# ignacio-rocco/detectorch

Hardware: AMD Instinct MI355X
Metric: images/sec Mask R-CNN R-50-FPN 1333x800 (region-proposal hot path) (higher is better)
Workload: dtype f32

## Files before the change

detectorch_amd/csrc/roi_align.hip:

```cpp
#include <stdlib.h>

#include <type_traits>

#include "roi_align_common.h"

namespace dtc {

constexpr int kRoiAlignThreads = 256;
constexpr int kMaxTableEntries = 2048;

__device__ __forceinline__ void build_axis_tables(AxisEntry* tab, const RoiHead& hd, const dtc_feat_level& L, int ny, int nx,
                                                  int ymul = 1, int xmul = 1) {
  for (int t = threadIdx.x; t < ny + nx; t += kRoiAlignThreads) {
    const bool is_y = t < ny;
    const int u = is_y ? t : t - ny, g = is_y ? hd.gh : hd.gw, mul = is_y ? ymul : xmul;
    AxisEntry e = make_axis(is_y ? hd.sh : hd.sw, is_y ? hd.bin_h : hd.bin_w, u / g, u % g, g, is_y ? L.height : L.width);
    e.lo *= mul; e.hi *= mul;
    tab[t] = e;
  }
}

template <typename TIn, typename TOut, bool FROM_TABLE>
__device__ __forceinline__ void gather_outputs(const RoiHead& hd, const dtc_feat_level& L, const AxisEntry* ytab, const AxisEntry* xtab,
                                               const TIn* base, TOut* out, int nc, int pooled_w, int bins) {
// ... 503 lines not shown
      } else {
      for (int iy = 0; iy < gh; iy++) {
        const AxisEntry y = tab_ok ? ytab[ph * gh + iy] : [&] { AxisEntry e = make_axis(sh, bin_h, ph, iy, gh, L.height); e.lo *= (int)L.stride_h; e.hi *= (int)L.stride_h; return e; }();
        for (int ix = 0; ix < gw; ix++) {
          const AxisEntry x = tab_ok ? xtab[pw * gw + ix] : [&] { AxisEntry e = make_axis(sw, bin_w, pw, ix, gw, L.width); e.lo *= (int)L.stride_w; e.hi *= (int)L.stride_w; return e; }();
          const float w1 = y.h * x.h, w2 = y.h * x.l, w3 = y.l * x.h, w4 = y.l * x.l;
          float4 v1, v2, v3, v4;
          if (vec) {
            v1 = load4(base + y.lo + x.lo); v2 = load4(base + y.lo + x.hi);
            v3 = load4(base + y.hi + x.lo); v4 = load4(base + y.hi + x.hi);
          } else {
            const TIn* t1 = base + y.lo + x.lo; const TIn* t2 = base + y.lo + x.hi;
            const TIn* t3 = base + y.hi + x.lo; const TIn* t4 = base + y.hi + x.hi;
            const int nv = nc - 4 * q;
            v1 = make_float4(to_f32<TIn>(t1[0]), nv > 1 ? to_f32<TIn>(t1[1]) : 0.f, nv > 2 ? to_f32<TIn>(t1[2]) : 0.f, nv > 3 ? to_f32<TIn>(t1[3]) : 0.f);
            v2 = make_float4(to_f32<TIn>(t2[0]), nv > 1 ? to_f32<TIn>(t2[1]) : 0.f, nv > 2 ? to_f32<TIn>(t2[2]) : 0.f, nv > 3 ? to_f32<TIn>(t2[3]) : 0.f);
            v3 = make_float4(to_f32<TIn>(t3[0]), nv > 1 ? to_f32<TIn>(t3[1]) : 0.f, nv > 2 ? to_f32<TIn>(t3[2]) : 0.f, nv > 3 ? to_f32<TIn>(t3[3]) : 0.f);
            v4 = make_float4(to_f32<TIn>(t4[0]), nv > 1 ? to_f32<TIn>(t4[1]) : 0.f, nv > 2 ? to_f32<TIn>(t4[2]) : 0.f, nv > 3 ? to_f32<TIn>(t4[3]) : 0.f);
          }
          a0 += w1 * v1.x + w2 * v2.x + w3 * v3.x + w4 * v4.x;
          a1 += w1 * v1.y + w2 * v2.y + w3 * v3.y + w4 * v4.y;
          a2 += w1 * v1.z + w2 * v2.z + w3 * v3.z + w4 * v4.z;
          a3 += w1 * v1.w + w2 * v2.w + w3 * v3.w + w4 * v4.w;
        }
      }
      }
      float* so = slab + (4 * q) * bins + bin;
      if (inv_count != 0.f) { so[0] = a0 * inv_count; so[bins] = a1 * inv_count; so[2 * bins] = a2 * inv_count; so[3 * bins] = a3 * inv_count; }
      else { so[0] = fdiv(a0, count); so[bins] = fdiv(a1, count); so[2 * bins] = fdiv(a2, count); so[3 * bins] = fdiv(a3, count); }
    }
  }
  __syncthreads();
  store_slab_vec<TOut, kRoiAlignThreads>(out, slab, nc * bins, tid);
}

const RoiAlignKnobs& roi_align_knobs() {
  static const RoiAlignKnobs knobs = [] {
    RoiAlignKnobs k;
    const auto first_not_0 = [](const char* name, bool dflt) { const char* e = getenv(name); return e ? e[0] != '0' : dflt; };
    const auto is_set = [](const char* name) { return getenv(name) != nullptr; };
    const auto number = [](const char* name, int dflt) { const char* e = getenv(name); return e ? atoi(e) : dflt; };
    const auto in_range = [&](const char* name, int lo, int hi, int dflt) { const int v = number(name, dflt); return v >= lo && v <= hi ? v : dflt; };
    k.tile = first_not_0("DTC_ROIALIGN_TILE", true);
    k.map = first_not_0("DTC_ROIALIGN_MAP", true);
    k.general = is_set("DTC_ROIALIGN_GENERAL");
    k.nhwc_direct = !is_set("DTC_ROIALIGN_NO_NHWC_DIRECT");
    k.nhwc16 = first_not_0("DTC_RA_NHWC16", true);
    k.nhwc_direct32 = first_not_0("DTC_RA_NHWC_DIRECT32", true);
    k.xcd = !is_set("DTC_RA_NO_XCD");
    k.cts64 = !is_set("DTC_RA_NO_CTS64");
    const int cb = number("DTC_RA_TILE_CHBLOCK", 0);
    if (cb >= 4 && (cb & 3) == 0) k.tile_ch_block = cb;
    k.tile_cb_major = number("DTC_RA_TILE_CBMAJOR", 1) != 0;
    k.tile_lds16_kb = in_range("DTC_RA_TILE_LDS16_KB", 36, 156, 0);
    k.map_prep = number("DTC_RA_MAP_PREP", 1) != 0;
    k.map_pitch = first_not_0("DTC_RA_MAP_PITCH", true);
    k.nhwc_lds = number("DTC_RA_NHWC_LDS", 1) != 0;
    k.nhwc_lds_kb = in_range("DTC_RA_NHWC_LDS_KB", 24, 160, 0);
    k.nhwc_pipe = in_range("DTC_RA_NHWC_PIPE", 0, 2, 1);
    return k;
  }();
  return knobs;
}

constexpr int kLdsKernelBytes = 52 * 1024;

template <typename TIn, typename TOut, int CB>
static int launch_nhwc_cb(const RoiAlignParams& p, hipStream_t stream) {
  const size_t smem = (size_t)kLdsTableFloats * 4 + (size_t)CB * p.pooled_h * p.pooled_w * 4 + 16;
  if (raise_lds_once<roi_align_fwd_nhwc<TIn, TOut, CB>>() != DTC_OK) return DTC_ELAUNCH;
  const int nct = ceil_div(p.channels, CB);
  hipLaunchKernelGGL((roi_align_fwd_nhwc<TIn, TOut, CB>), dim3((unsigned)p.n_rois * nct), dim3(kRoiAlignThreads), smem, stream, p);
  DTC_CHECK_LAUNCH();
  return DTC_OK;
}

template <typename TIn, typename TOut>
static int launch_nhwc(const RoiAlignParams& p, hipStream_t stream) {
  if (p.n_rois == 0) return DTC_OK;
  if constexpr (sizeof(TIn) == 2) {
    if (p.pooled_h * p.pooled_w > 64 && p.channels % 32 == 0) return launch_nhwc_cb<TIn, TOut, 32>(p, stream);
  }
  return launch_nhwc_cb<TIn, TOut, 64>(p, stream);
}

template <typename TIn, typename TOut>
static int launch_lds(const RoiAlignParams& p, hipStream_t stream) {
  if (p.n_rois == 0) return DTC_OK;
  if (raise_lds_once<roi_align_fwd_lds<TIn, TOut>>() != DTC_OK) return DTC_ELAUNCH;
  const int nct = ceil_div(p.channels, p.ch_block);
  hipLaunchKernelGGL((roi_align_fwd_lds<TIn, TOut>), dim3((unsigned)p.n_rois * nct), dim3(kRoiAlignThreads), kLdsKernelBytes, stream, p,
                     kLdsKernelBytes / 4);
  DTC_CHECK_LAUNCH();
  return DTC_OK;
}

template <typename TIn, typename TOut>
static int launch_general(const RoiAlignParams& p, hipStream_t stream) {
  if (p.n_rois == 0) return DTC_OK;
  int entries = p.sampling_ratio > 0 ? (p.pooled_h + p.pooled_w) * p.sampling_ratio : kMaxTableEntries;
  if (entries > kMaxTableEntries) entries = kMaxTableEntries;
  size_t smem = (size_t)entries * sizeof(AxisEntry);
  dim3 grid(p.n_rois, ceil_div(p.channels, p.ch_tile));
  hipLaunchKernelGGL((roi_align_fwd_general<TIn, TOut>), grid, dim3(kRoiAlignThreads), smem, stream, p);
  DTC_CHECK_LAUNCH();
  return DTC_OK;
// ... 102 lines not shown
```

detectorch_amd/csrc/roi_align_common.h:

```cpp
#pragma once
#include "dtc_common.h"
#include "wave_ops.h"

namespace dtc {

struct RoiAlignParams {
  dtc_feat_level lv[DTC_MAX_LEVELS];
  const float* rois;
  const int32_t* roi_levels;
  const int32_t* roi_order;
  const float* roi_desc;
  void* out;
  int n_levels, channels, roi_cols, n_rois, pooled_h, pooled_w, sampling_ratio, ch_tile;
  int ch_block;
  int cts64;
  int xcd_remap;
  const void* prep = nullptr;
};

constexpr int kXcds = 8;
__device__ __forceinline__ int xcd_work_item(int b, int n, int enabled) {
  if (!enabled || n < 2 * kXcds) return b;
  const int x = b % kXcds, j = b / kXcds;
  const int q = n / kXcds, r = n - q * kXcds;
// ... 94 lines not shown
  const f32x2 w2 = {w, w};
  acc = __builtin_elementwise_fma(v, w2, acc);
}
template <> __device__ __forceinline__ void fma_pair16<float>(f32x2&, uint32_t, float) {}

__device__ __forceinline__ float4 load4(const float* p) { return *reinterpret_cast<const float4*>(p); }
__device__ __forceinline__ float4 load4(const __half* p) { return f16x4_to_f32(*reinterpret_cast<const uint2*>(p)); }
__device__ __forceinline__ float4 load4(const bf16_t* p) { return bf16x4_to_f32(*reinterpret_cast<const uint2*>(p)); }

template <typename TOut> __device__ __forceinline__ void store4(TOut* d, float4 v);
template <> __device__ __forceinline__ void store4<float>(float* d, float4 v) { store_stream16(d, v); }
template <> __device__ __forceinline__ void store4<__half>(__half* d, float4 v) {
  const __half2 a = __floats2half2_rn(v.x, v.y), b = __floats2half2_rn(v.z, v.w);
  store_stream8(d, *reinterpret_cast<const uint32_t*>(&a), *reinterpret_cast<const uint32_t*>(&b));
}
template <> __device__ __forceinline__ void store4<bf16_t>(bf16_t* d, float4 v) {
  store_stream8(d, (uint32_t)from_f32<bf16_t>(v.x).bits | ((uint32_t)from_f32<bf16_t>(v.y).bits << 16),
                (uint32_t)from_f32<bf16_t>(v.z).bits | ((uint32_t)from_f32<bf16_t>(v.w).bits << 16));
}

template <typename TOut, int THREADS>
__device__ __forceinline__ void zero_outputs(TOut* out, int n, int tid) {
  for (int o = tid; o < n; o += THREADS) out[o] = from_f32<TOut>(0.f);
}

template <typename T> struct dtype_tag { typedef T type; };
template <typename Tag> using tag_type = typename Tag::type;
template <typename F>
inline int dispatch_io_pair(int in_dtype, int out_dtype, F&& f) {
  if (in_dtype == DTC_F32 && out_dtype == DTC_F32) return f(dtype_tag<float>{}, dtype_tag<float>{});
  if (in_dtype == DTC_F16 && out_dtype == DTC_F32) return f(dtype_tag<__half>{}, dtype_tag<float>{});
  if (in_dtype == DTC_F16 && out_dtype == DTC_F16) return f(dtype_tag<__half>{}, dtype_tag<__half>{});
  if (in_dtype == DTC_F32 && out_dtype == DTC_F16) return f(dtype_tag<float>{}, dtype_tag<__half>{});
  if (in_dtype == DTC_BF16 && out_dtype == DTC_F32) return f(dtype_tag<bf16_t>{}, dtype_tag<float>{});
  if (in_dtype == DTC_BF16 && out_dtype == DTC_BF16) return f(dtype_tag<bf16_t>{}, dtype_tag<bf16_t>{});
  if (in_dtype == DTC_F32 && out_dtype == DTC_BF16) return f(dtype_tag<float>{}, dtype_tag<bf16_t>{});
  return DTC_EUNSUPPORTED;
}
inline bool io_pair_supported(int in_dtype, int out_dtype) {
  return dispatch_io_pair(in_dtype, out_dtype, [](auto, auto) { return (int)DTC_OK; }) == DTC_OK;
}

struct RoiAlignKnobs {
  bool tile = true;
  bool map = true;
  bool general = false;
  bool nhwc_direct = true;
  bool nhwc16 = true;
  bool nhwc_direct32 = true;
  bool xcd = true;
  bool cts64 = true;
  int tile_ch_block = 0;
  int tile_cb_major = 1;
  int tile_lds16_kb = 0;
  bool map_prep = true;
  bool map_pitch = true;
  int nhwc_lds = 1;
  int nhwc_lds_kb = 0;
  int nhwc_pipe = 1;
};
const RoiAlignKnobs& roi_align_knobs();

bool roi_align_tile_supported(const RoiAlignParams& p, int in_dtype, int out_dtype);
int launch_roi_align_tile(const RoiAlignParams& p, int in_dtype, int out_dtype, hipStream_t stream);
bool roi_align_map_supported(const RoiAlignParams& p, int in_dtype, int out_dtype);
int launch_roi_align_map(const RoiAlignParams& p, int in_dtype, int out_dtype, hipStream_t stream);
void roi_align_set_exact(int exact);
int roi_align_get_exact();
size_t roi_align_map_workspace_bytes(int n_rois);
int launch_roi_align_map_ws(const RoiAlignParams& p, int in_dtype, int out_dtype, void* workspace, size_t workspace_bytes, hipStream_t stream);

bool roi_align_nhwc_lds_supported(const RoiAlignParams& p, int in_dtype, int out_dtype);
int launch_roi_align_nhwc_lds(const RoiAlignParams& p, int in_dtype, int out_dtype, hipStream_t stream);

bool roi_align_nhwc16_supported(const RoiAlignParams& p, int in_dtype, int out_dtype);
int launch_roi_align_nhwc16(const RoiAlignParams& p, int in_dtype, int out_dtype, hipStream_t stream);

}
```

detectorch_amd/csrc/roi_align_tile.hip:

```cpp

#include <type_traits>

#include "roi_align_common.h"

namespace dtc {

constexpr int kTileMaxK = 32;
constexpr int kTileRoiBytes = 48, kTileGroupBytes = 32;
constexpr int kTileHdrBytes = kTileMaxK * (kTileRoiBytes + kTileGroupBytes) + 16;
template <int NT> struct TileShape;
template <> struct TileShape<256> { static constexpr int kUnits = 8, kWaves = 3, kLdsKB = 52, kWaves16 = 4, kLds16KB = 38; };

struct TileRoi {
  int lvl, b, x0, x1, y0, y1, r, valid;
  float sh, sw, bin_h, bin_w;
};
static_assert(sizeof(TileRoi) == kTileRoiBytes, "TileRoi layout");
struct TileGroup { int first, count, kind, x0, x1, y0, y1, pad; };
enum { kGrpPool = 0, kGrpZero = 1, kGrpAbsent = 2, kGrpGather = 3 };

__device__ __forceinline__ __amdgpu_buffer_rsrc_t make_srd(const void* base) {
  return __builtin_amdgcn_make_buffer_rsrc(const_cast<void*>(base), 0, 0xffffffff, 0x00020000);
}
template <typename TIn> struct Piece4;
template <> struct Piece4<float> {
  typedef float4 Raw;
  static __device__ __forceinline__ Raw raw(__amdgpu_buffer_rsrc_t r, uint32_t voff, uint32_t soff) {
    const u32x4 v = __builtin_amdgcn_raw_buffer_load_b128(r, voff, soff, 0);
    return make_float4(__uint_as_float(v.x), __uint_as_float(v.y), __uint_as_float(v.z), __uint_as_float(v.w));
  }
};
template <> struct Piece4<__half> {
  typedef u32x2 Raw;
  static __device__ __forceinline__ Raw raw(__amdgpu_buffer_rsrc_t r, uint32_t voff, uint32_t soff) { return __builtin_amdgcn_raw_buffer_load_b64(r, voff, soff, 0); }
};
template <> struct Piece4<bf16_t> {
  typedef u32x2 Raw;
  static __device__ __forceinline__ Raw raw(__amdgpu_buffer_rsrc_t r, uint32_t voff, uint32_t soff) { return __builtin_amdgcn_raw_buffer_load_b64(r, voff, soff, 0); }
};

template <typename TIn> struct TileLds { typedef float T; static constexpr int kSlot = 16, kShift = 4; };
template <> struct TileLds<__half> { typedef uint16_t T; static constexpr int kSlot = 8, kShift = 3; };
template <> struct TileLds<bf16_t> { typedef uint16_t T; static constexpr int kSlot = 8, kShift = 3; };

template <typename TIn, int NT> struct TileBounds { static constexpr int kWaves = TileShape<NT>::kWaves; };
template <int NT> struct TileBounds<__half, NT> { static constexpr int kWaves = TileShape<NT>::kWaves16; };
template <int NT> struct TileBounds<bf16_t, NT> { static constexpr int kWaves = TileShape<NT>::kWaves16; };

__device__ __forceinline__ int tile_phys(int px) { return px + (px >> 3); }

struct TileItem {
  int a[2][2][4];
  float yl[2], yh[2], xl[2], xh[2];
  bool on;
};

enum { kStageScalar = 0, kStageVec = 1, kStageVecUnaligned = 2 };

struct TileGeom {
  int first, count;
  int y0, x0a, ngx, npos;
  int plane;
  int nq_pass;
  int mode;
};

template <typename TIn, typename TOut, int NT, bool FUSED>
__device__ __forceinline__ void tile_passes(const RoiAlignParams& p, const dtc_feat_level& L, const TIn* fbase, int c0, int nc,
                                            int bins, float* slab, typename TileLds<TIn>::T* win, const TileRoi* troi, const TileGeom& g,
                                            const TileItem& it, int rl, int bin) {
  constexpr int NW = NT / 64;
  constexpr int U = TileShape<NT>::kUnits;
  typedef typename TileLds<TIn>::T TL;
  constexpr bool L16 = sizeof(TL) == 2;
  constexpr int SB = TileLds<TIn>::kSlot;
  const int tid = threadIdx.x, lane = tid & 63, wv = tid >> 6, pl = lane & 15, cl = (lane >> 4) & 3;
  const int npos = g.npos, ngx = g.ngx, plane = g.plane, nq_pass = g.nq_pass;
  const int nchunk = (npos + 15) >> 4;
  const int KC = ceil_div(nchunk, NW);
  const float rinv = 1.0f / (float)ngx;
  const int nq_tot = ceil_div(nc, 4);
  const bool vec = g.mode != kStageScalar;
  uint32_t uoff[U];
  int ulds[U];
  const int nu = KC * nq_pass;
  if (vec) {
    const int sh32 = (int)L.stride_h, sc32 = (int)L.stride_c;
    int q = 0, i = 0;
#pragma unroll
    for (int u = 0; u < U; u++) {
      const bool dup = u >= nu;
      const int pos = min((wv + (dup ? 0 : i) * NW) * 16 + pl, npos - 1);
      const int row = (int)(((float)pos + 0.5f) * rinv);
      const int gx = pos - row * ngx;
      const int qq = dup ? 0 : q;
      int col = g.x0a + 4 * gx, sft = 0;
      if (g.mode == kStageVecUnaligned) { sft = max(0, col + 3 - (L.width - 1)); col -= sft; }
      uoff[u] = ((uint32_t)((g.y0 + row) * sh32 + col + (4 * qq + cl) * sc32) * (uint32_t)sizeof(TIn)) | ((uint32_t)sft << 30);
      ulds[u] = qq * plane * 4 + ((4 * pos + (pos >> 1)) << 2) + cl;
      if (++i == KC) { i = 0; q++; }
    }
  }
  const __amdgpu_buffer_rsrc_t srd = make_srd(fbase);
  const uint32_t pass_bytes = (uint32_t)(L.stride_c * (int64_t)sizeof(TIn));
  typename Piece4<TIn>::Raw v[U];
  auto issue = [&](int cs) {
    const uint32_t soff = (uint32_t)cs * pass_bytes;
    if (g.mode == kStageVec) {
#pragma unroll
      for (int u = 0; u < U; u++) v[u] = Piece4<TIn>::raw(srd, uoff[u], soff);
    } else {
#pragma unroll
      for (int u = 0; u < U; u++) v[u] = Piece4<TIn>::raw(srd, uoff[u] & 0x3fffffffu, soff);
    }
  };
  auto commit_as = [&](auto shifted_tag) {
    constexpr bool SHIFTED = decltype(shifted_tag)::value;
    if constexpr (SHIFTED) asm volatile("" ::: "memory");
#pragma unroll
    for (int u = 0; u < U; u++) {
      if constexpr (L16) {
        uint32_t w0 = v[u].x & 0xffffu, w1 = v[u].x >> 16, w2 = v[u].y & 0xffffu, w3 = v[u].y >> 16;
        if constexpr (SHIFTED) {
// ... 29 lines not shown
      const int cq = cs + 4 * q;
      if (cq >= nc) break;
      const int cle = min(cl, nc - 1 - cq);
      const TIn* base = fbase + (int64_t)(cq + cle) * L.stride_c;
#pragma unroll 1
      for (int t = wv; t < nchunk; t += NW) {
        const int pos = min(t * 16 + pl, npos - 1);
        const int row = (int)(((float)pos + 0.5f) * rinv);
        const int gx = pos - row * ngx;
        const int rem = L.width - 1 - (g.x0a + 4 * gx);
        const TIn* s = base + (int64_t)(g.y0 + row) * L.stride_h + (int64_t)(g.x0a + 4 * gx) * L.stride_w;
        TL* d = win + q * plane * 4 + ((4 * pos + (pos >> 1)) << 2) + cl;
        d[0] = lds_val(s[0]);
        d[4] = lds_val(s[(int64_t)min(1, rem) * L.stride_w]);
        d[8] = lds_val(s[(int64_t)min(2, rem) * L.stride_w]);
        d[12] = lds_val(s[(int64_t)min(3, rem) * L.stride_w]);
      }
    }
  };
  const bool quad_ok = ((p.channels | c0) & 3) == 0;
  auto store_slab = [&](int cs, int nq) {
    const int nch = min(4 * nq, nc - cs);
    TOut* out = reinterpret_cast<TOut*>(p.out);
    if (quad_ok && nch == 4 * nq) {
      const int n4 = nq * bins, total = g.count * n4;
      const float r4 = 1.0f / (float)n4;
      const int cs_off = cs * bins;
      for (int idx = tid; idx < total; idx += NT) {
        const int k = (int)(((float)idx + 0.5f) * r4);
        const int e = idx - __mul24(k, n4);
        const float4 val = reinterpret_cast<const float4*>(slab)[idx];
        const uint64_t ob = *reinterpret_cast<const uint64_t*>(&troi[g.first + k].x0);
        store4<TOut>(out + (ob + (uint64_t)(uint32_t)(cs_off + 4 * e)), val);
      }
    } else {
      const int per = nch * bins, total = g.count * per;
      for (int idx = tid; idx < total; idx += NT) {
        const int k = idx / per, e = idx - k * per;
        out[((size_t)troi[g.first + k].r * p.channels + c0 + cs) * bins + e] = from_f32<TOut>(slab[k * 4 * nq * bins + e]);
      }
    }
  };

  if (vec) issue(0);
  int cs_prev = 0, nq_prev = 0;
#pragma unroll 1
  for (int qs = 0; qs < nq_tot; qs += nq_pass) {
    const int cs = 4 * qs;
    const int nq_cur = min(nq_pass, nq_tot - qs);
    if (vec) commit(); else stage_scalar(cs);
    if (nq_prev) store_slab(cs_prev, nq_prev);
    __syncthreads();
    if (vec && qs + nq_pass < nq_tot) issue(cs + 4 * nq_pass);
    if (it.on) {
      float* so = slab + rl * (4 * nq_cur * bins) + bin;
#pragma unroll 1
      for (int q = 0; q < nq_cur; q++) {
        const char* wq = reinterpret_cast<const char*>(win) + uni(q * plane * SB);
        f32x2 a01 = {0.f, 0.f}, a23 = {0.f, 0.f};
#pragma unroll
        for (int iy = 0; iy < 2; iy++) {
          if constexpr (L16 && FUSED) {
            u32x2 t[2][4];
#pragma unroll
            for (int ix = 0; ix < 2; ix++)
#pragma unroll
              for (int k = 0; k < 4; k++)
                t[ix][k] = *reinterpret_cast<const u32x2*>(__builtin_assume_aligned(wq + it.a[iy][ix][k], 8));
#pragma unroll
            for (int ix = 0; ix < 2; ix++) {
              const float w1 = it.yh[iy] * it.xh[ix], w2 = it.yh[iy] * it.xl[ix];
              const float w3 = it.yl[iy] * it.xh[ix], w4 = it.yl[iy] * it.xl[ix];
              fma_pair16<TIn>(a01, t[ix][0].x, w1); fma_pair16<TIn>(a23, t[ix][0].y, w1);
              fma_pair16<TIn>(a01, t[ix][1].x, w2); fma_pair16<TIn>(a23, t[ix][1].y, w2);
              fma_pair16<TIn>(a01, t[ix][2].x, w3); fma_pair16<TIn>(a23, t[ix][2].y, w3);
              fma_pair16<TIn>(a01, t[ix][3].x, w4); fma_pair16<TIn>(a23, t[ix][3].y, w4);
            }
          } else if constexpr (L16) {
            u32x2 t[2][4];
#pragma unroll
            for (int ix = 0; ix < 2; ix++)
#pragma unroll
              for (int k = 0; k < 4; k++)
                t[ix][k] = *reinterpret_cast<const u32x2*>(__builtin_assume_aligned(wq + it.a[iy][ix][k], 8));
#pragma unroll
            for (int ix = 0; ix < 2; ix++) {
              const float w1 = it.yh[iy] * it.xh[ix], w2 = it.yh[iy] * it.xl[ix];
              const float w3 = it.yl[iy] * it.xh[ix], w4 = it.yl[iy] * it.xl[ix];
              f32x2 s01 = mul_pair16<TIn>(t[ix][0].x, w1) + mul_pair16<TIn>(t[ix][1].x, w2);
              s01 = s01 + mul_pair16<TIn>(t[ix][2].x, w3);
              s01 = s01 + mul_pair16<TIn>(t[ix][3].x, w4);
              f32x2 s23 = mul_pair16<TIn>(t[ix][0].y, w1) + mul_pair16<TIn>(t[ix][1].y, w2);
              s23 = s23 + mul_pair16<TIn>(t[ix][2].y, w3);
              s23 = s23 + mul_pair16<TIn>(t[ix][3].y, w4);
              a01 = a01 + s01; a23 = a23 + s23;
            }
          } else {
            f32x4 t[2][4];
#pragma unroll
            for (int ix = 0; ix < 2; ix++)
#pragma unroll
              for (int k = 0; k < 4; k++)
                t[ix][k] = *reinterpret_cast<const f32x4*>(__builtin_assume_aligned(wq + it.a[iy][ix][k], 16));
#pragma unroll
            for (int ix = 0; ix < 2; ix++) {
              const float w1 = it.yh[iy] * it.xh[ix], w2 = it.yh[iy] * it.xl[ix];
              const float w3 = it.yl[iy] * it.xh[ix], w4 = it.yl[iy] * it.xl[ix];
              a01 += w1 * t[ix][0].lo + w2 * t[ix][1].lo + w3 * t[ix][2].lo + w4 * t[ix][3].lo;
              a23 += w1 * t[ix][0].hi + w2 * t[ix][1].hi + w3 * t[ix][2].hi + w4 * t[ix][3].hi;
            }
          }
          __builtin_amdgcn_sched_barrier(0);
        }
        float* o = so + uni(4 * q * bins);
        const float a0 = a01.x, a1 = a01.y, a2 = a23.x, a3 = a23.y;
        o[0] = a0 * 0.25f; o[bins] = a1 * 0.25f; o[2 * bins] = a2 * 0.25f; o[3 * bins] = a3 * 0.25f;
      }
    }
    __syncthreads();
    cs_prev = cs; nq_prev = nq_cur;
  }
  if (nq_prev) store_slab(cs_prev, nq_prev);
}

__device__ __forceinline__ int tile_work_item(int b, int n, int reverse) {
  if (n < 2 * kXcds || (reverse & 2)) return (reverse & 1) ? n - 1 - b : b;
  const int x = b % kXcds, j = b / kXcds;
  const int q = n / kXcds, r = n - q * kXcds;
  const int start = x * q + min(x, r), qx = q + (x < r ? 1 : 0);
  return start + ((reverse & 1) ? qx - 1 - j : j);
}

template <typename TIn, typename TOut, int NT, bool FUSED>
__global__ __launch_bounds__(NT, (TileBounds<TIn, NT>::kWaves)) void roi_align_fwd_tile(RoiAlignParams p, int kgroup, int lds_bytes, int nq_cap, int merge_pct, int reverse) {
  extern __shared__ __attribute__((aligned(16))) unsigned char smem[];
  TileRoi* troi = reinterpret_cast<TileRoi*>(smem);
  TileGroup* tgrp = reinterpret_cast<TileGroup*>(smem + kTileMaxK * kTileRoiBytes);
  int* ngp = reinterpret_cast<int*>(smem + kTileMaxK * (kTileRoiBytes + kTileGroupBytes));
  const int slab_bytes = kgroup * p.pooled_h * p.pooled_w * 16 * nq_cap;
  float* slab = reinterpret_cast<float*>(smem + kTileHdrBytes);
  typedef typename TileLds<TIn>::T TL;
  constexpr int SB = TileLds<TIn>::kSlot;
  TL* win = reinterpret_cast<TL*>(smem + kTileHdrBytes + slab_bytes);
  const int win_bytes = lds_bytes - kTileHdrBytes - slab_bytes;
  constexpr int NW = NT / 64;
  constexpr int kMaxPos = TileShape<NT>::kUnits * NW * 16;
  const int tid = threadIdx.x;
  const int nct = ceil_div(p.channels, p.ch_block);
  const int wi = tile_work_item(blockIdx.x, gridDim.x, reverse);
  int grp = wi / nct;
  int c0 = (wi - grp * nct) * p.ch_block;
  {
    const int ngrp = (int)gridDim.x / nct;
    if ((reverse & 4) && ngrp % kXcds == 0 && ngrp >= 2 * kXcds) {
      const int x = blockIdx.x % kXcds, j = blockIdx.x / kXcds, ngx = ngrp / kXcds;
      const int cbi = j / ngx, gl = j - cbi * ngx;
      grp = x * ngx + ((reverse & 1) ? ngx - 1 - gl : gl);
      c0 = cbi * p.ch_block;
    }
  }
  const int nc = min(p.ch_block, p.channels - c0);
  const int bins = p.pooled_h * p.pooled_w;
  const int K = kgroup;

  if (tid < 64) {
    TileRoi t;
    t.lvl = -1; t.b = 0; t.x0 = t.x1 = t.y0 = t.y1 = 0; t.r = 0; t.valid = 0; t.sh = t.sw = 0.f; t.bin_h = t.bin_w = 1.f;
    const int ri = grp * K + tid;
    if (tid < K && ri < p.n_rois) {
      const RoiHead hd = load_roi_head(p, ri);
      t.valid = 1; t.r = hd.r; t.b = hd.b; t.sh = hd.sh; t.sw = hd.sw; t.bin_h = hd.bin_h; t.bin_w = hd.bin_w;
      if (hd.lvl >= 0 && hd.lvl < p.n_levels) {
        t.lvl = hd.lvl;
        const int H = p.lv[hd.lvl].height, W = p.lv[hd.lvl].width;
        t.y0 = make_axis(hd.sh, hd.bin_h, 0, 0, 2, H).lo;
        t.y1 = make_axis(hd.sh, hd.bin_h, p.pooled_h - 1, 1, 2, H).hi;
        t.x0 = make_axis(hd.sw, hd.bin_w, 0, 0, 2, W).lo;
        t.x1 = make_axis(hd.sw, hd.bin_w, p.pooled_w - 1, 1, 2, W).hi;
      }
    }
    if (tid < K) {
      troi[tid] = t;
      *reinterpret_cast<uint64_t*>(&troi[tid].x0) = ((uint64_t)(uint32_t)t.r * (uint64_t)p.channels + (uint64_t)c0) * (uint64_t)(p.pooled_h * p.pooled_w);
    }
    auto bc = [](int v, int k) { return __builtin_amdgcn_readlane(v, k); };
    int ng = 0, k = 0;
    while (k < K) {
      const int ks = uni(k);
      const int a_lvl = bc(t.lvl, ks), a_b = bc(t.b, ks), a_valid = bc(t.valid, ks);
      const int a_x0 = bc(t.x0, ks), a_x1 = bc(t.x1, ks), a_y0 = bc(t.y0, ks), a_y1 = bc(t.y1, ks);
      TileGroup g;
      g.first = k; g.count = 1; g.x0 = a_x0; g.x1 = a_x1; g.y0 = a_y0; g.y1 = a_y1; g.pad = 0;
      if (!a_valid) g.kind = kGrpAbsent;
      else if (a_lvl < 0) g.kind = kGrpZero;
      else {
        const int ngx0 = (a_x1 >> 2) - (a_x0 >> 2) + 1, th0 = a_y1 - a_y0 + 1, npos0 = th0 * ngx0;
        if (npos0 > kMaxPos || (4 * npos0 + (npos0 >> 1) + 1) * SB > win_bytes || bins > NT) {
          g.kind = kGrpGather;
        } else {
          g.kind = kGrpPool;
          long long sum_px = (long long)th0 * (a_x1 - a_x0 + 1);
          while (k + g.count < K && (g.count + 1) * bins <= NT) {
            const int js = uni(k + g.count);
            const int n_lvl = bc(t.lvl, js), n_b = bc(t.b, js), n_valid = bc(t.valid, js);
            if (!n_valid || n_lvl != a_lvl || n_b != a_b) break;
            const int n_x0 = bc(t.x0, js), n_x1 = bc(t.x1, js), n_y0 = bc(t.y0, js), n_y1 = bc(t.y1, js);
            const int ux0 = min(g.x0, n_x0), ux1 = max(g.x1, n_x1), uy0 = min(g.y0, n_y0), uy1 = max(g.y1, n_y1);
            const int ungx = (ux1 >> 2) - (ux0 >> 2) + 1, uth = uy1 - uy0 + 1, unpos = uth * ungx;
            if (unpos > kMaxPos || (4 * unpos + (unpos >> 1) + 1) * SB > win_bytes) break;
            const long long n_px = (long long)(n_y1 - n_y0 + 1) * (n_x1 - n_x0 + 1);
            const long long u_px = (long long)uth * (ux1 - ux0 + 1);
            if (u_px * 100 > (sum_px + n_px) * merge_pct) break;
            g.x0 = ux0; g.x1 = ux1; g.y0 = uy0; g.y1 = uy1; g.count++;
            sum_px += n_px;
          }
        }
      }
      if (tid == 0) tgrp[ng] = g;
      ng++;
      k += g.count;
    }
    if (tid == 0) *ngp = ng;
  }
  __syncthreads();

  const int ngroups = uni(*ngp);
  for (int gi = 0; gi < ngroups; gi++) {
    const int first = uni(tgrp[gi].first), count = uni(tgrp[gi].count), kind = uni(tgrp[gi].kind);
    if (kind == kGrpAbsent) continue;
    if (kind == kGrpZero) {
      TOut* oz = reinterpret_cast<TOut*>(p.out) + ((size_t)uni(troi[first].r) * p.channels + c0) * bins;
      zero_outputs<TOut, NT>(oz, nc * bins, tid);
      continue;
    }
    const int lvl = uni(troi[first].lvl), b = uni(troi[first].b);
    const dtc_feat_level L = p.lv[lvl];
    const TIn* fbase = reinterpret_cast<const TIn*>(L.data) + (int64_t)b * L.stride_n + (int64_t)c0 * L.stride_c;
    if (kind == kGrpGather) {
      const RoiHead hd = load_roi_head(p, grp * K + first);
      TOut* og = reinterpret_cast<TOut*>(p.out) + ((size_t)hd.r * p.channels + c0) * bins;
      for (int o = tid; o < nc * bins; o += NT) {
        const int c = o / bins, bin = o - c * bins;
        const int ph = bin / p.pooled_w, pw = bin - ph * p.pooled_w;
        const TIn* d = fbase + (int64_t)c * L.stride_c;
        float acc = 0.f;
        for (int iy = 0; iy < 2; iy++) {
          const AxisEntry y = make_axis(hd.sh, hd.bin_h, ph, iy, 2, L.height);
          const int64_t ylo = (int64_t)y.lo * L.stride_h, yhi = (int64_t)y.hi * L.stride_h;
          for (int ix = 0; ix < 2; ix++) {
            const AxisEntry x = make_axis(hd.sw, hd.bin_w, pw, ix, 2, L.width);
            const int64_t xlo = (int64_t)x.lo * L.stride_w, xhi = (int64_t)x.hi * L.stride_w;
            const float w1 = y.h * x.h, w2 = y.h * x.l, w3 = y.l * x.h, w4 = y.l * x.l;
            acc += w1 * to_f32<TIn>(d[ylo + xlo]) + w2 * to_f32<TIn>(d[ylo + xhi]) + w3 * to_f32<TIn>(d[yhi + xlo]) +
                   w4 * to_f32<TIn>(d[yhi + xhi]);
          }
        }
        og[o] = from_f32<TOut>(acc * 0.25f);
      }
      continue;
    }
    const int gx0 = uni(tgrp[gi].x0), gx1 = uni(tgrp[gi].x1), gy0 = uni(tgrp[gi].y0), gy1 = uni(tgrp[gi].y1);
    TileGeom g;
    g.first = first; g.count = count;
    g.y0 = gy0; g.x0a = gx0 & ~3;
    g.ngx = (gx1 >> 2) - (gx0 >> 2) + 1;
    const int tw = 4 * g.ngx, th = gy1 - gy0 + 1;
    g.npos = th * g.ngx;
    g.plane = 4 * g.npos + (g.npos >> 1) + 1;
    const int esz = (int)sizeof(TIn);
    const bool lin = L.stride_w == 1 && ((nc | c0) & 3) == 0 && L.stride_h > 0 && L.stride_c > 0 &&
                     L.stride_h * L.height + L.stride_c * 4 * TileShape<NT>::kUnits < (1ll << 26);
    const bool al16 = ((L.width | L.stride_h | L.stride_c | L.stride_n) & 3) == 0 &&
                      (reinterpret_cast<uintptr_t>(L.data) & (4 * sizeof(TIn) - 1)) == 0;
    const bool al4 = L.width >= 4 && (((L.width | L.stride_h | L.stride_c | L.stride_n) * esz) & 3) == 0 &&
                     (reinterpret_cast<uintptr_t>(L.data) & 3) == 0;
    g.mode = !lin ? kStageScalar : al16 ? kStageVec : al4 ? kStageVecUnaligned : kStageScalar;
    const int KC = ceil_div((g.npos + 15) >> 4, NW);
    g.nq_pass = max(1, min(min(win_bytes / (g.plane * SB), TileShape<NT>::kUnits / KC), min(ceil_div(nc, 4), nq_cap)));
    while (ceil_div(nc, 4) % g.nq_pass) g.nq_pass--;
    const int n_it = count * bins;
    TileItem it;
    it.on = tid < n_it;
    const int itx = it.on ? tid : 0;
    const int rl = itx / bins, bin = itx - rl * bins;
    const int ph = bin / p.pooled_w, pw = bin - ph * p.pooled_w;
    const TileRoi hd = troi[first + rl];
    int ylo[2], yhi[2], xlo[2], xhi[2];
#pragma unroll
    for (int i = 0; i < 2; i++) {
      const AxisEntry ey = make_axis(hd.sh, hd.bin_h, ph, i, 2, L.height);
      const AxisEntry ex = make_axis(hd.sw, hd.bin_w, pw, i, 2, L.width);
      it.yl[i] = ey.l; it.yh[i] = ey.h; it.xl[i] = ex.l; it.xh[i] = ex.h;
      ylo[i] = (ey.lo - gy0) * tw; yhi[i] = (ey.hi - gy0) * tw;
      xlo[i] = ex.lo - g.x0a; xhi[i] = ex.hi - g.x0a;
    }
#pragma unroll
    for (int iy = 0; iy < 2; iy++)
#pragma unroll
      for (int ix = 0; ix < 2; ix++) {
        constexpr int SS = TileLds<TIn>::kShift;
        int t0 = tile_phys(ylo[iy] + xlo[ix]) << SS, t1 = tile_phys(ylo[iy] + xhi[ix]) << SS;
        int t2 = tile_phys(yhi[iy] + xlo[ix]) << SS, t3 = tile_phys(yhi[iy] + xhi[ix]) << SS;
        asm volatile("" : "+v"(t0), "+v"(t1), "+v"(t2), "+v"(t3));
        it.a[iy][ix][0] = t0; it.a[iy][ix][1] = t1; it.a[iy][ix][2] = t2; it.a[iy][ix][3] = t3;
      }
    tile_passes<TIn, TOut, NT, FUSED>(p, L, fbase, c0, nc, bins, slab, win, troi, g, it, rl, bin);
  }
}

constexpr int kTileThreads = 256;
constexpr int kTileMergePct = 250;
constexpr int kTileNqCap = 4;
constexpr int kTileReverse = 1;

template <typename TIn, typename TOut, int NT, bool FUSED>
static int launch_tile_nt(RoiAlignParams p, hipStream_t stream) {
  const RoiAlignKnobs& cfg = roi_align_knobs();
  const int bins = p.pooled_h * p.pooled_w;
  int K = NT / bins;
  K = K < 1 ? 1 : (K > kTileMaxK ? kTileMaxK : K);
  if (K * bins > NT) K = NT / bins;
  if (K < 1) return DTC_EUNSUPPORTED;
  const int lds_b = (sizeof(TIn) == 2 ? (cfg.tile_lds16_kb ? cfg.tile_lds16_kb : TileShape<NT>::kLds16KB) : TileShape<NT>::kLdsKB) * 1024;
  if (raise_lds_once<roi_align_fwd_tile<TIn, TOut, NT, FUSED>>() != DTC_OK) return DTC_ELAUNCH;
  const int nq_cap = kTileNqCap;
  if (kTileHdrBytes + K * bins * 16 * nq_cap + 20 * 1024 > lds_b) return DTC_EUNSUPPORTED;
  const int ngrp = ceil_div(p.n_rois, K);
  int cb = cfg.tile_ch_block ? cfg.tile_ch_block : ((long long)ngrp * ceil_div(p.channels, 128) >= 6144 ? 128 : 64);
  while (!cfg.tile_ch_block && cb > 32 && (long long)ngrp * ceil_div(p.channels, cb) < 2048) cb >>= 1;
  p.ch_block = cb;
  const int nct = ceil_div(p.channels, p.ch_block);
  hipLaunchKernelGGL((roi_align_fwd_tile<TIn, TOut, NT, FUSED>), dim3((unsigned)ngrp * nct), dim3(NT), lds_b, stream, p, K, lds_b, nq_cap, kTileMergePct, (kTileReverse ? 1 : 0) | (p.xcd_remap ? 0 : 2) | (cfg.tile_cb_major ? 4 : 0));
  DTC_CHECK_LAUNCH();
  return DTC_OK;
}

template <typename TIn, typename TOut>
static int launch_tile_t(const RoiAlignParams& p, hipStream_t stream) {
  if constexpr (sizeof(TIn) == 2) { if (!roi_align_get_exact()) return launch_tile_nt<TIn, TOut, kTileThreads, true>(p, stream); }
  return launch_tile_nt<TIn, TOut, kTileThreads, false>(p, stream);
}

bool roi_align_tile_supported(const RoiAlignParams& p, int in_dtype, int out_dtype) {
  if (p.sampling_ratio != 2) return false;
  if (p.pooled_h * p.pooled_w > kTileThreads) return false;
  return io_pair_supported(in_dtype, out_dtype);
}

int launch_roi_align_tile(const RoiAlignParams& p, int in_dtype, int out_dtype, hipStream_t stream) {
  if (p.n_rois == 0) return DTC_OK;
  return dispatch_io_pair(in_dtype, out_dtype, [&](auto tin, auto tout) {
    return launch_tile_t<tag_type<decltype(tin)>, tag_type<decltype(tout)>>(p, stream);
  });
}

}
```

Before: 14850.

## Process two ROI items per thread in fp32 tile RoIAlign kernel

For fp32 input, the tile kernel now assigns two ROI bin items to each thread (RND=2). K doubles per block so more ROIs share one staged LDS feature window, and nq_cap is halved to stay within LDS. LDS tap offsets are packed as 16-bit pairs to save registers, and weights are computed with an inline multiply that carries an LDS-address dependency. The group-clustering logic moves into a shared tile_plan.h header. The intent is more reuse of each staged window and fewer blocks, at the cost of extra registers and fewer channel quads per pass.

```diff
diff --git a/detectorch_amd/csrc/roi_align.hip b/detectorch_amd/csrc/roi_align.hip
--- a/detectorch_amd/csrc/roi_align.hip
+++ b/detectorch_amd/csrc/roi_align.hip
@@ -579,6 +579,7 @@
     const int cb = number("DTC_RA_TILE_CHBLOCK", 0);
     if (cb >= 4 && (cb & 3) == 0) k.tile_ch_block = cb;
     k.tile_cb_major = number("DTC_RA_TILE_CBMAJOR", 1) != 0;
+    k.tile_pair = first_not_0("DTC_RA_TILE_PAIR", true);
     k.tile_lds16_kb = in_range("DTC_RA_TILE_LDS16_KB", 36, 156, 0);
     k.map_prep = number("DTC_RA_MAP_PREP", 1) != 0;
     k.map_pitch = first_not_0("DTC_RA_MAP_PITCH", true);
diff --git a/detectorch_amd/csrc/roi_align_common.h b/detectorch_amd/csrc/roi_align_common.h
--- a/detectorch_amd/csrc/roi_align_common.h
+++ b/detectorch_amd/csrc/roi_align_common.h
@@ -170,6 +170,7 @@
   bool cts64 = true;
   int tile_ch_block = 0;
   int tile_cb_major = 1;
+  bool tile_pair = true;
   int tile_lds16_kb = 0;
   bool map_prep = true;
   bool map_pitch = true;
diff --git a/detectorch_amd/csrc/roi_align_tile.hip b/detectorch_amd/csrc/roi_align_tile.hip
--- a/detectorch_amd/csrc/roi_align_tile.hip
+++ b/detectorch_amd/csrc/roi_align_tile.hip
@@ -2,6 +2,7 @@
 #include <type_traits>
 
 #include "roi_align_common.h"
+#include "tile_plan.h"
 
 namespace dtc {
 
@@ -16,8 +17,7 @@
   float sh, sw, bin_h, bin_w;
 };
 static_assert(sizeof(TileRoi) == kTileRoiBytes, "TileRoi layout");
-struct TileGroup { int first, count, kind, x0, x1, y0, y1, pad; };
-enum { kGrpPool = 0, kGrpZero = 1, kGrpAbsent = 2, kGrpGather = 3 };
+static_assert(sizeof(TileGroup) == kTileGroupBytes, "TileGroup layout");
 
 __device__ __forceinline__ __amdgpu_buffer_rsrc_t make_srd(const void* base) {
   return __builtin_amdgcn_make_buffer_rsrc(const_cast<void*>(base), 0, 0xffffffff, 0x00020000);
@@ -53,7 +53,28 @@
   int a[2][2][4];
   float yl[2], yh[2], xl[2], xh[2];
   bool on;
-};
+  __device__ __forceinline__ int tap(int iy, int ix, int k) const { return a[iy][ix][k]; }
+};
+struct TileItemHalf {
+  uint32_t a2[2][2][2];
+  float yl[2], yh[2], xl[2], xh[2];
+  bool on;
+  __device__ __forceinline__ uint32_t tap_at(uint32_t base, int iy, int ix, int k) const {
+    uint32_t r;
+    if (k & 1) asm("v_add_u32_sdwa %0, %1, %2 dst_sel:DWORD dst_unused:UNUSED_PAD src0_sel:DWORD src1_sel:WORD_1" : "=v"(r) : "s"(base), "v"(a2[iy][ix][k >> 1]));
+    else asm("v_add_u32_sdwa %0, %1, %2 dst_sel:DWORD dst_unused:UNUSED_PAD src0_sel:DWORD src1_sel:WORD_0" : "=v"(r) : "s"(base), "v"(a2[iy][ix][k >> 1]));
+    return r;
+  }
+};
+typedef __attribute__((address_space(3))) unsigned char lds_byte;
+typedef __attribute__((address_space(3))) const f32x4 lds_f32x4;
+__device__ __forceinline__ float mul_in_turn(float a, float b, uint32_t turn) {
+  float r;
+  asm("v_mul_f32 %0, %1, %2" : "=v"(r) : "v"(a), "v"(b), "s"(turn));
+  return r;
+}
+template <int RND> struct TileItems { TileItem it[1]; };
+template <> struct TileItems<2> { TileItemHalf it[2]; };
 
 enum { kStageScalar = 0, kStageVec = 1, kStageVecUnaligned = 2 };
 
@@ -65,10 +86,10 @@
   int mode;
 };
 
-template <typename TIn, typename TOut, int NT, bool FUSED>
+template <typename TIn, typename TOut, int NT, bool FUSED, int RND>
 __device__ __forceinline__ void tile_passes(const RoiAlignParams& p, const dtc_feat_level& L, const TIn* fbase, int c0, int nc,
                                             int bins, float* slab, typename TileLds<TIn>::T* win, const TileRoi* troi, const TileGeom& g,
-                                            const TileItem& it, int rl, int bin) {
+                                            const TileItems<RND>& its, int rl, int per, int bin) {
   constexpr int NW = NT / 64;
   constexpr int U = TileShape<NT>::kUnits;
   typedef typename TileLds<TIn>::T TL;
@@ -204,11 +225,13 @@
     if (nq_prev) store_slab(cs_prev, nq_prev);
     __syncthreads();
     if (vec && qs + nq_pass < nq_tot) issue(cs + 4 * nq_pass);
-    if (it.on) {
-      float* so = slab + rl * (4 * nq_cur * bins) + bin;
+    auto pool = [&](const auto& it, int rli) {
+      float* so = slab + rli * (4 * nq_cur * bins) + bin;
 #pragma unroll 1
       for (int q = 0; q < nq_cur; q++) {
         const char* wq = reinterpret_cast<const char*>(win) + uni(q * plane * SB);
+        [[maybe_unused]] uint32_t wqa = 0;
+        if constexpr (RND == 2) wqa = (uint32_t)uni((int)((uint32_t)(uintptr_t)(lds_byte*)win + (uint32_t)(q * plane * SB)));
         f32x2 a01 = {0.f, 0.f}, a23 = {0.f, 0.f};
 #pragma unroll
         for (int iy = 0; iy < 2; iy++) {
@@ -218,7 +241,7 @@
             for (int ix = 0; ix < 2; ix++)
 #pragma unroll
               for (int k = 0; k < 4; k++)
-                t[ix][k] = *reinterpret_cast<const u32x2*>(__builtin_assume_aligned(wq + it.a[iy][ix][k], 8));
+                t[ix][k] = *reinterpret_cast<const u32x2*>(__builtin_assume_aligned(wq + it.tap(iy, ix, k), 8));
 #pragma unroll
             for (int ix = 0; ix < 2; ix++) {
               const float w1 = it.yh[iy] * it.xh[ix], w2 = it.yh[iy] * it.xl[ix];
@@ -234,7 +257,7 @@
             for (int ix = 0; ix < 2; ix++)
 #pragma unroll
               for (int k = 0; k < 4; k++)
-                t[ix][k] = *reinterpret_cast<const u32x2*>(__builtin_assume_aligned(wq + it.a[iy][ix][k], 8));
+                t[ix][k] = *reinterpret_cast<const u32x2*>(__builtin_assume_aligned(wq + it.tap(iy, ix, k), 8));
 #pragma unroll
             for (int ix = 0; ix < 2; ix++) {
               const float w1 = it.yh[iy] * it.xh[ix], w2 = it.yh[iy] * it.xl[ix];
@@ -252,12 +275,19 @@
 #pragma unroll
             for (int ix = 0; ix < 2; ix++)
 #pragma unroll
-              for (int k = 0; k < 4; k++)
-                t[ix][k] = *reinterpret_cast<const f32x4*>(__builtin_assume_aligned(wq + it.a[iy][ix][k], 16));
+              for (int k = 0; k < 4; k++) {
+                if constexpr (RND == 1) t[ix][k] = *reinterpret_cast<const f32x4*>(__builtin_assume_aligned(wq + it.tap(iy, ix, k), 16));
+                else t[ix][k] = *(lds_f32x4*)(uintptr_t)it.tap_at(wqa, iy, ix, k);
+              }
 #pragma unroll
             for (int ix = 0; ix < 2; ix++) {
-              const float w1 = it.yh[iy] * it.xh[ix], w2 = it.yh[iy] * it.xl[ix];
-              const float w3 = it.yl[iy] * it.xh[ix], w4 = it.yl[iy] * it.xl[ix];
+              float w1, w2, w3, w4;
+              if constexpr (RND == 1) {
+                w1 = it.yh[iy] * it.xh[ix]; w2 = it.yh[iy] * it.xl[ix]; w3 = it.yl[iy] * it.xh[ix]; w4 = it.yl[iy] * it.xl[ix];
+              } else {
+                w1 = mul_in_turn(it.yh[iy], it.xh[ix], wqa); w2 = mul_in_turn(it.yh[iy], it.xl[ix], wqa);
+                w3 = mul_in_turn(it.yl[iy], it.xh[ix], wqa); w4 = mul_in_turn(it.yl[iy], it.xl[ix], wqa);
+              }
               a01 += w1 * t[ix][0].lo + w2 * t[ix][1].lo + w3 * t[ix][2].lo + w4 * t[ix][3].lo;
               a23 += w1 * t[ix][0].hi + w2 * t[ix][1].hi + w3 * t[ix][2].hi + w4 * t[ix][3].hi;
             }
@@ -268,7 +298,10 @@
         const float a0 = a01.x, a1 = a01.y, a2 = a23.x, a3 = a23.y;
         o[0] = a0 * 0.25f; o[bins] = a1 * 0.25f; o[2 * bins] = a2 * 0.25f; o[3 * bins] = a3 * 0.25f;
       }
-    }
+    };
+#pragma unroll
+    for (int r = 0; r < RND; r++)
+      if (its.it[r].on) pool(its.it[r], rl + r * per);
     __syncthreads();
     cs_prev = cs; nq_prev = nq_cur;
   }
@@ -283,7 +316,7 @@
   return start + ((reverse & 1) ? qx - 1 - j : j);
 }
 
-template <typename TIn, typename TOut, int NT, bool FUSED>
+template <typename TIn, typename TOut, int NT, bool FUSED, int RND>
 __global__ __launch_bounds__(NT, (TileBounds<TIn, NT>::kWaves)) void roi_align_fwd_tile(RoiAlignParams p, int kgroup, int lds_bytes, int nq_cap, int merge_pct, int reverse) {
   extern __shared__ __attribute__((aligned(16))) unsigned char smem[];
   TileRoi* troi = reinterpret_cast<TileRoi*>(smem);
@@ -336,38 +369,17 @@
       *reinterpret_cast<uint64_t*>(&troi[tid].x0) = ((uint64_t)(uint32_t)t.r * (uint64_t)p.channels + (uint64_t)c0) * (uint64_t)(p.pooled_h * p.pooled_w);
     }
     auto bc = [](int v, int k) { return __builtin_amdgcn_readlane(v, k); };
+    const TilePlanRules rules = {K, bins, RND * NT, NT, kMaxPos, win_bytes, SB, merge_pct};
+    auto win_of = [&](int j) {
+      const int js = uni(j);
+      TileWin w;
+      w.lvl = bc(t.lvl, js); w.b = bc(t.b, js); w.valid = bc(t.valid, js);
+      w.x0 = bc(t.x0, js); w.x1 = bc(t.x1, js); w.y0 = bc(t.y0, js); w.y1 = bc(t.y1, js);
+      return w;
+    };
     int ng = 0, k = 0;
     while (k < K) {
-      const int ks = uni(k);
-      const int a_lvl = bc(t.lvl, ks), a_b = bc(t.b, ks), a_valid = bc(t.valid, ks);
-      const int a_x0 = bc(t.x0, ks), a_x1 = bc(t.x1, ks), a_y0 = bc(t.y0, ks), a_y1 = bc(t.y1, ks);
-      TileGroup g;
-      g.first = k; g.count = 1; g.x0 = a_x0; g.x1 = a_x1; g.y0 = a_y0; g.y1 = a_y1; g.pad = 0;
-      if (!a_valid) g.kind = kGrpAbsent;
-      else if (a_lvl < 0) g.kind = kGrpZero;
-      else {
-        const int ngx0 = (a_x1 >> 2) - (a_x0 >> 2) + 1, th0 = a_y1 - a_y0 + 1, npos0 = th0 * ngx0;
-        if (npos0 > kMaxPos || (4 * npos0 + (npos0 >> 1) + 1) * SB > win_bytes || bins > NT) {
-          g.kind = kGrpGather;
-        } else {
-          g.kind = kGrpPool;
-          long long sum_px = (long long)th0 * (a_x1 - a_x0 + 1);
-          while (k + g.count < K && (g.count + 1) * bins <= NT) {
-            const int js = uni(k + g.count);
-            const int n_lvl = bc(t.lvl, js), n_b = bc(t.b, js), n_valid = bc(t.valid, js);
-            if (!n_valid || n_lvl != a_lvl || n_b != a_b) break;
-            const int n_x0 = bc(t.x0, js), n_x1 = bc(t.x1, js), n_y0 = bc(t.y0, js), n_y1 = bc(t.y1, js);
-            const int ux0 = min(g.x0, n_x0), ux1 = max(g.x1, n_x1), uy0 = min(g.y0, n_y0), uy1 = max(g.y1, n_y1);
-            const int ungx = (ux1 >> 2) - (ux0 >> 2) + 1, uth = uy1 - uy0 + 1, unpos = uth * ungx;
-            if (unpos > kMaxPos || (4 * unpos + (unpos >> 1) + 1) * SB > win_bytes) break;
-            const long long n_px = (long long)(n_y1 - n_y0 + 1) * (n_x1 - n_x0 + 1);
-            const long long u_px = (long long)uth * (ux1 - ux0 + 1);
-            if (u_px * 100 > (sum_px + n_px) * merge_pct) break;
-            g.x0 = ux0; g.x1 = ux1; g.y0 = uy0; g.y1 = uy1; g.count++;
-            sum_px += n_px;
-          }
-        }
-      }
+      const TileGroup g = tile_plan_cluster(k, rules, win_of);
       if (tid == 0) tgrp[ng] = g;
       ng++;
       k += g.count;
@@ -430,33 +442,45 @@
     const int KC = ceil_div((g.npos + 15) >> 4, NW);
     g.nq_pass = max(1, min(min(win_bytes / (g.plane * SB), TileShape<NT>::kUnits / KC), min(ceil_div(nc, 4), nq_cap)));
     while (ceil_div(nc, 4) % g.nq_pass) g.nq_pass--;
-    const int n_it = count * bins;
-    TileItem it;
-    it.on = tid < n_it;
-    const int itx = it.on ? tid : 0;
+    const int per = K / RND;
+    const int n_it = min(count, per) * bins;
+    const bool lane_on = tid < n_it;
+    const int itx = lane_on ? tid : 0;
     const int rl = itx / bins, bin = itx - rl * bins;
     const int ph = bin / p.pooled_w, pw = bin - ph * p.pooled_w;
-    const TileRoi hd = troi[first + rl];
-    int ylo[2], yhi[2], xlo[2], xhi[2];
-#pragma unroll
-    for (int i = 0; i < 2; i++) {
-      const AxisEntry ey = make_axis(hd.sh, hd.bin_h, ph, i, 2, L.height);
-      const AxisEntry ex = make_axis(hd.sw, hd.bin_w, pw, i, 2, L.width);
-      it.yl[i] = ey.l; it.yh[i] = ey.h; it.xl[i] = ex.l; it.xh[i] = ex.h;
-      ylo[i] = (ey.lo - gy0) * tw; yhi[i] = (ey.hi - gy0) * tw;
-      xlo[i] = ex.lo - g.x0a; xhi[i] = ex.hi - g.x0a;
-    }
-#pragma unroll
-    for (int iy = 0; iy < 2; iy++)
-#pragma unroll
-      for (int ix = 0; ix < 2; ix++) {
-        constexpr int SS = TileLds<TIn>::kShift;
-        int t0 = tile_phys(ylo[iy] + xlo[ix]) << SS, t1 = tile_phys(ylo[iy] + xhi[ix]) << SS;
-        int t2 = tile_phys(yhi[iy] + xlo[ix]) << SS, t3 = tile_phys(yhi[iy] + xhi[ix]) << SS;
-        asm volatile("" : "+v"(t0), "+v"(t1), "+v"(t2), "+v"(t3));
-        it.a[iy][ix][0] = t0; it.a[iy][ix][1] = t1; it.a[iy][ix][2] = t2; it.a[iy][ix][3] = t3;
-      }
-    tile_passes<TIn, TOut, NT, FUSED>(p, L, fbase, c0, nc, bins, slab, win, troi, g, it, rl, bin);
+    TileItems<RND> its;
+#pragma unroll
+    for (int r = 0; r < RND; r++) {
+      auto& it = its.it[r];
+      it.on = lane_on && (RND == 1 || rl + r * per < count);
+      const TileRoi hd = troi[first + (it.on ? rl + r * per : 0)];
+      int ylo[2], yhi[2], xlo[2], xhi[2];
+#pragma unroll
+      for (int i = 0; i < 2; i++) {
+        const AxisEntry ey = make_axis(hd.sh, hd.bin_h, ph, i, 2, L.height);
+        const AxisEntry ex = make_axis(hd.sw, hd.bin_w, pw, i, 2, L.width);
+        it.yl[i] = ey.l; it.yh[i] = ey.h; it.xl[i] = ex.l; it.xh[i] = ex.h;
+        ylo[i] = (ey.lo - gy0) * tw; yhi[i] = (ey.hi - gy0) * tw;
+        xlo[i] = ex.lo - g.x0a; xhi[i] = ex.hi - g.x0a;
+      }
+#pragma unroll
+      for (int iy = 0; iy < 2; iy++)
+#pragma unroll
+        for (int ix = 0; ix < 2; ix++) {
+          constexpr int SS = TileLds<TIn>::kShift;
+          int t0 = tile_phys(ylo[iy] + xlo[ix]) << SS, t1 = tile_phys(ylo[iy] + xhi[ix]) << SS;
+          int t2 = tile_phys(yhi[iy] + xlo[ix]) << SS, t3 = tile_phys(yhi[iy] + xhi[ix]) << SS;
+          if constexpr (RND == 1) {
+            asm volatile("" : "+v"(t0), "+v"(t1), "+v"(t2), "+v"(t3));
+            it.a[iy][ix][0] = t0; it.a[iy][ix][1] = t1; it.a[iy][ix][2] = t2; it.a[iy][ix][3] = t3;
+          } else {
+            uint32_t h0 = ((uint32_t)t0 & 0xffffu) | ((uint32_t)t1 << 16), h1 = ((uint32_t)t2 & 0xffffu) | ((uint32_t)t3 << 16);
+            asm volatile("" : "+v"(h0), "+v"(h1));
+            it.a2[iy][ix][0] = h0; it.a2[iy][ix][1] = h1;
+          }
+        }
+    }
+    tile_passes<TIn, TOut, NT, FUSED, RND>(p, L, fbase, c0, nc, bins, slab, win, troi, g, its, rl, per, bin);
   }
 }
 
@@ -465,32 +489,39 @@
 constexpr int kTileNqCap = 4;
 constexpr int kTileReverse = 1;
 
-template <typename TIn, typename TOut, int NT, bool FUSED>
+template <typename TIn, typename TOut, int NT, bool FUSED, int RND>
 static int launch_tile_nt(RoiAlignParams p, hipStream_t stream) {
   const RoiAlignKnobs& cfg = roi_align_knobs();
   const int bins = p.pooled_h * p.pooled_w;
   int K = NT / bins;
-  K = K < 1 ? 1 : (K > kTileMaxK ? kTileMaxK : K);
+  K = K < 1 ? 1 : (K > kTileMaxK / RND ? kTileMaxK / RND : K);
   if (K * bins > NT) K = NT / bins;
   if (K < 1) return DTC_EUNSUPPORTED;
+  K *= RND;
   const int lds_b = (sizeof(TIn) == 2 ? (cfg.tile_lds16_kb ? cfg.tile_lds16_kb : TileShape<NT>::kLds16KB) : TileShape<NT>::kLdsKB) * 1024;
-  if (raise_lds_once<roi_align_fwd_tile<TIn, TOut, NT, FUSED>>() != DTC_OK) return DTC_ELAUNCH;
-  const int nq_cap = kTileNqCap;
+  if (raise_lds_once<roi_align_fwd_tile<TIn, TOut, NT, FUSED, RND>>() != DTC_OK) return DTC_ELAUNCH;
+  const int nq_cap = kTileNqCap / RND;
   if (kTileHdrBytes + K * bins * 16 * nq_cap + 20 * 1024 > lds_b) return DTC_EUNSUPPORTED;
   const int ngrp = ceil_div(p.n_rois, K);
-  int cb = cfg.tile_ch_block ? cfg.tile_ch_block : ((long long)ngrp * ceil_div(p.channels, 128) >= 6144 ? 128 : 64);
-  while (!cfg.tile_ch_block && cb > 32 && (long long)ngrp * ceil_div(p.channels, cb) < 2048) cb >>= 1;
+  const long long nunit = (long long)ngrp * RND;
+  int cb = cfg.tile_ch_block ? cfg.tile_ch_block : (nunit * ceil_div(p.channels, 128) >= 6144 ? 128 : 64);
+  while (!cfg.tile_ch_block && cb > 32 && nunit * ceil_div(p.channels, cb) < 2048) cb >>= 1;
   p.ch_block = cb;
   const int nct = ceil_div(p.channels, p.ch_block);
-  hipLaunchKernelGGL((roi_align_fwd_tile<TIn, TOut, NT, FUSED>), dim3((unsigned)ngrp * nct), dim3(NT), lds_b, stream, p, K, lds_b, nq_cap, kTileMergePct, (kTileReverse ? 1 : 0) | (p.xcd_remap ? 0 : 2) | (cfg.tile_cb_major ? 4 : 0));
+  hipLaunchKernelGGL((roi_align_fwd_tile<TIn, TOut, NT, FUSED, RND>), dim3((unsigned)ngrp * nct), dim3(NT), lds_b, stream, p, K, lds_b, nq_cap, kTileMergePct, (kTileReverse ? 1 : 0) | (p.xcd_remap ? 0 : 2) | (cfg.tile_cb_major ? 4 : 0));
   DTC_CHECK_LAUNCH();
   return DTC_OK;
 }
 
 template <typename TIn, typename TOut>
 static int launch_tile_t(const RoiAlignParams& p, hipStream_t stream) {
-  if constexpr (sizeof(TIn) == 2) { if (!roi_align_get_exact()) return launch_tile_nt<TIn, TOut, kTileThreads, true>(p, stream); }
-  return launch_tile_nt<TIn, TOut, kTileThreads, false>(p, stream);
+  if constexpr (sizeof(TIn) == 2) { if (!roi_align_get_exact()) return launch_tile_nt<TIn, TOut, kTileThreads, true, 1>(p, stream); }
+  if constexpr (std::is_same<TIn, float>::value) {
+    const int bins = p.pooled_h * p.pooled_w;
+    if (roi_align_knobs().tile_pair && 2 * bins <= kTileThreads && 2 * (kTileThreads / bins) <= kTileMaxK)
+      return launch_tile_nt<TIn, TOut, kTileThreads, false, 2>(p, stream);
+  }
+  return launch_tile_nt<TIn, TOut, kTileThreads, false, 1>(p, stream);
 }
 
 bool roi_align_tile_supported(const RoiAlignParams& p, int in_dtype, int out_dtype) {
diff --git a/detectorch_amd/csrc/tile_plan.h b/detectorch_amd/csrc/tile_plan.h
--- /dev/null
+++ b/detectorch_amd/csrc/tile_plan.h
@@ -0,0 +1,60 @@
+#pragma once
+
+#if defined(__HIPCC__)
+#define DTC_PLAN_HD __host__ __device__ __forceinline__
+#else
+#define DTC_PLAN_HD inline
+#endif
+
+namespace dtc {
+
+struct TileGroup { int first, count, kind, x0, x1, y0, y1, pad; };
+enum { kGrpPool = 0, kGrpZero = 1, kGrpAbsent = 2, kGrpGather = 3 };
+enum { kCutEnd = 0, kCutLanes = 1, kCutOther = 2, kCutPieces = 3, kCutImage = 4, kCutArea = 5 };
+
+struct TileWin { int lvl, b, valid, x0, x1, y0, y1; };
+
+struct TilePlanRules {
+  int K;
+  int bins;
+  int lanes;
+  int threads;
+  int max_pos;
+  int win_bytes;
+  int slot_bytes;
+  int merge_pct;
+};
+
+DTC_PLAN_HD int tile_plan_min(int a, int b) { return a < b ? a : b; }
+DTC_PLAN_HD int tile_plan_max(int a, int b) { return a > b ? a : b; }
+DTC_PLAN_HD int tile_plan_slots(int npos) { return 4 * npos + (npos >> 1) + 1; }
+
+template <typename Win>
+DTC_PLAN_HD TileGroup tile_plan_cluster(int k, const TilePlanRules& R, Win win) {
+  const TileWin a = win(k);
+  TileGroup g;
+  g.first = k; g.count = 1; g.x0 = a.x0; g.x1 = a.x1; g.y0 = a.y0; g.y1 = a.y1; g.pad = kCutEnd;
+  if (!a.valid) { g.kind = kGrpAbsent; return g; }
+  if (a.lvl < 0) { g.kind = kGrpZero; return g; }
+  const int ngx0 = (a.x1 >> 2) - (a.x0 >> 2) + 1, th0 = a.y1 - a.y0 + 1, npos0 = th0 * ngx0;
+  if (npos0 > R.max_pos || tile_plan_slots(npos0) * R.slot_bytes > R.win_bytes || R.bins > R.threads) { g.kind = kGrpGather; return g; }
+  g.kind = kGrpPool;
+  long long sum_px = (long long)th0 * (a.x1 - a.x0 + 1);
+  while (k + g.count < R.K) {
+    if ((g.count + 1) * R.bins > R.lanes) { g.pad = kCutLanes; break; }
+    const TileWin n = win(k + g.count);
+    if (!n.valid || n.lvl != a.lvl || n.b != a.b) { g.pad = kCutOther; break; }
+    const int ux0 = tile_plan_min(g.x0, n.x0), ux1 = tile_plan_max(g.x1, n.x1), uy0 = tile_plan_min(g.y0, n.y0), uy1 = tile_plan_max(g.y1, n.y1);
+    const int ungx = (ux1 >> 2) - (ux0 >> 2) + 1, uth = uy1 - uy0 + 1, unpos = uth * ungx;
+    if (unpos > R.max_pos) { g.pad = kCutPieces; break; }
+    if (tile_plan_slots(unpos) * R.slot_bytes > R.win_bytes) { g.pad = kCutImage; break; }
+    const long long n_px = (long long)(n.y1 - n.y0 + 1) * (n.x1 - n.x0 + 1);
+    const long long u_px = (long long)uth * (ux1 - ux0 + 1);
+    if (u_px * 100 > (sum_px + n_px) * R.merge_pct) { g.pad = kCutArea; break; }
+    g.x0 = ux0; g.x1 = ux1; g.y0 = uy0; g.y1 = uy1; g.count++;
+    sum_px += n_px;
+  }
+  return g;
+}
+
+}
```

Result: slower. 14680 (-1.1%).
